# huawei-noah/xingtian

Measured on NVIDIA H100. Metric: learner env-steps/sec (Atari 84x84x4 PPO), higher is better.
Workload: dtype f32 (bf16x3 split on wgmma, fp32 accumulate in registers)

## Files before the change

include/xtb200.h:

```cpp
#ifndef XTB200_H_
#define XTB200_H_

#include <stddef.h>
#include <stdint.h>

#ifdef __cplusplus
extern "C" {
#endif

#define XTB_VERSION 101

enum xtb_status {
  XTB_OK = 0,
  XTB_ERR_ARG = -1,
  XTB_ERR_CUDA = -2,
  XTB_ERR_STATE = -3,
  XTB_ERR_NOMEM = -4
};

enum xtb_layer_kind { XTB_CONV = 0, XTB_DENSE = 1, XTB_DUELING = 2, XTB_LOGSTD = 3 };
enum xtb_act {
  XTB_ACT_NONE = 0, XTB_ACT_RELU = 1, XTB_ACT_TANH = 2, XTB_ACT_SIGMOID = 3, XTB_ACT_SOFTSIGN = 4, XTB_ACT_SOFTPLUS = 5,
  XTB_ACT_LEAKY_RELU = 6, XTB_ACT_ELU = 7, XTB_ACT_SELU = 8, XTB_ACT_SWISH = 9, XTB_ACT_GELU = 10
};
// ... 66 lines not shown
typedef struct xtb_ppo_hyper {
  float clip_ratio;
  float ent_coef;
  float vf_clip;
  float critic_coef;
} xtb_ppo_hyper;
int xtb_ppo_loss_grad(const float* logits, const float* v, const int32_t* gather_idx,
                      const int32_t* action, const float* old_logp, const float* adv,
                      const float* old_v, const float* target_v, int batch, int adim,
                      const xtb_ppo_hyper* hp, float inv_count, float* dlogits, float* dv,
                      float* loss_out, void* stream);

int xtb_vtrace_loss_grad(const float* tp_logits, const float* baseline, const float* bp_logits,
                         const int32_t* action, const uint8_t* done, const float* reward,
                         int n_traj, int step_len, int adim, float gamma, float* dlogits,
                         float* dbaseline, float* vs_out, float* pg_adv_out, float* loss_out,
                         void* stream);

int xtb_dqn_loss_grad(const float* q, const float* q_next_target, const float* q_next_online,
                      const int32_t* action, const float* reward, const uint8_t* done, int batch,
                      int adim, float gamma, float inv_count, float* dq, float* y_out,
                      float* loss_out, void* stream);

int xtb_dqn_td_loss_grad(const float* q, const float* q_next_target, const float* q_next_online, const int32_t* idx,
                         const int32_t* action, const float* reward, const uint8_t* done, const float* disc, int batch,
                         int adim, float gamma, float huber_delta, float inv_count, float* dq, float* y_out,
                         float* loss_out, void* stream);
int xtb_nstep_returns(const float* reward, const uint8_t* done, int n_env, int n_step, int n, float gamma, float* ret,
                      float* disc, int32_t* last, uint8_t* done_n, void* stream);

int xtb_mse_loss_grad(const float* q, const float* y, int batch, int adim, float inv_count, float* dq,
                      float* loss_out, void* stream);
int xtb_softmax(const float* logits, int batch, int adim, float* probs, void* stream);
int xtb_impala_keras_loss_grad(const float* logits, const float* v, const int32_t* idx, const float* action_mat,
                               const float* adv, const float* target_v, int batch, int adim, float ent_coef,
                               float value_weight, float loss_scale, float* dlogits, float* dv, float* loss_out,
                               void* stream);

typedef struct xtb_adam xtb_adam;
enum xtb_clip_mode { XTB_CLIP_NONE = 0, XTB_CLIP_GLOBAL_NORM = 1, XTB_CLIP_PER_TENSOR = 2 };
int xtb_adam_create(long long count, float lr, float beta1, float beta2, float eps, int clip_mode,
                    float clip, const long long* seg_offsets, int n_seg, float* m, float* v,
                    xtb_adam** out);
void xtb_adam_destroy(xtb_adam* opt);
int xtb_adam_step(xtb_adam* opt, float* params, const float* grads, float grad_scale, void* stream);
int xtb_adam_step_net(xtb_adam* opt, xtb_net* net, float grad_scale, void* stream);
const float* xtb_adam_grad_norm(const xtb_adam* opt);
int xtb_adam_set_lr(xtb_adam* opt, float lr);
int xtb_adam_set_decay(xtb_adam* opt, float decay);
int xtb_opt_use_rmsprop(xtb_adam* opt, float* mean_grad, float decay, float epsilon);
int xtb_opt_use_rmsprop_plain(xtb_adam* opt, float decay, float epsilon);

int xtb_ppo_heads_plan(const xtb_net* net, int pi_tensor, int v_tensor, int infer, int* kpl, int* amax);
typedef struct xtb_ppo_rollout {
  const void* obs;
  const void* action;
  const float* old_logp;
  const float* adv;
  const float* old_v;
  const float* target_v;
} xtb_ppo_rollout;
int xtb_ppo_train(xtb_net* net, xtb_adam* opt, const xtb_ppo_rollout* ro, int n_sample, int batch_size, int n_epoch,
                  const int32_t* perm, const xtb_ppo_hyper* hp, int pi_tensor, int v_tensor, int logstd_tensor,
                  float* loss_per_step, int use_graph, void* stream);

int xtb_impala_train(xtb_net* net, xtb_adam* opt, const void* obs, const int32_t* gather_idx, const float* bp_logits,
                     const int32_t* action, const uint8_t* done, const float* reward, int n_sample, int step_len,
                     float gamma, int logit_tensor, int base_tensor, float* loss_out, int use_graph, void* stream);
int xtb_dqn_train(xtb_net* net, xtb_net* target, xtb_adam* opt, const void* obs, const void* next_obs,
                  const int32_t* idx, const int32_t* action, const float* reward, const uint8_t* done,
                  const float* disc, int n_sample, float gamma, float huber_delta, int q_tensor, float* qn_t,
                  float* qn_o, float* loss_out, int use_graph, void* stream);

int xtb_impala_keras_fit(xtb_net* net, xtb_adam* opt, const void* obs, const int32_t* order, const float* action_mat,
                         const float* adv, const float* target_v, int n, int fit_batch, int logit_tensor, int v_tensor,
                         float ent_coef, float* loss_out, int use_graph, void* stream);
typedef struct xtb_impala_traj {
  const void* obs;
  const float* behav_prob;
  const float* action_mat;
  const float* reward;
  const uint8_t* done;
} xtb_impala_traj;
int xtb_impala_keras_train(xtb_net* net, xtb_adam* opt, const xtb_impala_traj* tr, int n_traj, int ep_len, int slice,
                           int fit_batch, const int32_t* order, int32_t* obs_idx, float gamma, float ent_coef,
                           int logit_tensor, int v_tensor, float* pg_adv, float* target_v, float* loss_per_slice,
                           int use_graph, void* stream);

int xtb_ppo_rollout_infer(xtb_net* net, const void* obs, const int32_t* step_idx, int n_env, int n_step, int pi_tensor,
                          int v_tensor, int logstd_tensor, uint64_t seed, unsigned long long* offset_dev, void* action,
                          float* logp, float* value, int use_graph, void* stream);

int xtb_ppo_predict_host(xtb_net* net, const void* obs_host, size_t obs_bytes, void* obs_dev, int n_env, int pi_tensor,
                         int v_tensor, int logstd_tensor, uint64_t seed, unsigned long long* offset_dev, float* out_dev,
                         float* out_host, float* head_host, int use_graph, void* stream);

int xtb_diag_gaussian_sample(const float* mean, const float* log_std, int batch, int adim, const float* normals,
                             uint64_t seed, uint64_t offset, float* action, float* logp, void* stream);
int xtb_ppo_gauss_loss_grad(const float* mean, const float* v, const float* log_std, const int32_t* gather_idx,
                            const float* action, const float* old_logp, const float* adv, const float* old_v,
                            const float* target_v, int batch, int adim, const xtb_ppo_hyper* hp, float inv_count,
                            float* dmean, float* dv, float* dlog_std, float* loss_out, void* stream);

typedef struct xtb_muzero xtb_muzero;
typedef struct xtb_muzero_desc {
  int32_t unroll;
// ... 117 lines not shown
```

xingtian_b200/capi.py:

```python
import ctypes as C
import os

HERE = os.path.dirname(os.path.abspath(__file__))
LIB_PATH = os.environ.get("XTB_LIB_PATH") or os.path.join(HERE, "lib", "libxtb200.so")

XTB_MAX_LAYERS = 16
CONV, DENSE, DUELING, LOGSTD = 0, 1, 2, 3
ACT = {None: 0, "linear": 0, "relu": 1, "tanh": 2, "sigmoid": 3, "softsign": 4, "softplus": 5, "leaky_relu": 6, "elu": 7,
       "selu": 8, "swish": 9, "gelu": 10}
CLIP_NONE, CLIP_GLOBAL_NORM, CLIP_PER_TENSOR = 0, 1, 2


class LayerDesc(C.Structure):
    _fields_ = [("kind", C.c_int32), ("src", C.c_int32), ("act", C.c_int32), ("k", C.c_int32),
                ("stride", C.c_int32), ("cout", C.c_int32), ("pad_same", C.c_int32)]


class NetDesc(C.Structure):
    _fields_ = [("input_u8", C.c_int32), ("scale", C.c_float), ("in_h", C.c_int32), ("in_w", C.c_int32),
                ("in_c", C.c_int32), ("n_layers", C.c_int32), ("layers", LayerDesc * XTB_MAX_LAYERS)]


class LayerPlan(C.Structure):
    _fields_ = [("kind", C.c_int32), ("tc", C.c_int32), ("s2d", C.c_int32), ("w_res", C.c_int32), ("n_fwd", C.c_int32),
# ... 59 lines not shown
    "xtb_net_param_count": (C.c_longlong, [_P]),
    "xtb_net_layer_params": (C.c_int, [_P, C.c_int, C.POINTER(C.c_longlong), C.POINTER(C.c_longlong),
                                       C.POINTER(C.c_int), C.POINTER(C.c_int)]),
    "xtb_net_layer_plan": (C.c_int, [_P, C.c_int, C.POINTER(LayerPlan)]),
    "xtb_net_tensor_size": (C.c_int, [_P, C.c_int]),
    "xtb_net_workspace_bytes": (C.c_size_t, [_P]),
    "xtb_net_bind": (C.c_int, [_P, _P, _P, _P, C.c_size_t]),
    "xtb_net_bind_stream": (C.c_int, [_P, _P, _P, _P, C.c_size_t, _P]),
    "xtb_net_sync_weights": (C.c_int, [_P, _P]),
    "xtb_net_tensor": (_P, [_P, C.c_int]),
    "xtb_net_tensor_grad": (_P, [_P, C.c_int]),
    "xtb_net_forward": (C.c_int, [_P, _P, _P, _P, C.c_int, _P]),
    "xtb_net_backward": (C.c_int, [_P, _P, _P, C.c_int, C.POINTER(C.c_int32), C.c_int, _P]),
    "xtb_categorical_sample": (C.c_int, [_P, C.c_int, C.c_int, _P, C.c_uint64, C.c_uint64, _P, _P, _P]),
    "xtb_argmax": (C.c_int, [_P, C.c_int, C.c_int, _P, _P]),
    "xtb_gae": (C.c_int, [_P, _P, _P, C.c_int, C.c_int, C.c_float, C.c_float, C.c_int, _P, _P, _P, _P]),
    "xtb_ppo_loss_grad": (C.c_int, [_P, _P, _P, _P, _P, _P, _P, _P, C.c_int, C.c_int, C.POINTER(PpoHyper),
                                    C.c_float, _P, _P, _P, _P]),
    "xtb_vtrace_loss_grad": (C.c_int, [_P, _P, _P, _P, _P, _P, C.c_int, C.c_int, C.c_int, C.c_float,
                                       _P, _P, _P, _P, _P, _P]),
    "xtb_dqn_loss_grad": (C.c_int, [_P, _P, _P, _P, _P, _P, C.c_int, C.c_int, C.c_float, C.c_float,
                                    _P, _P, _P, _P]),
    "xtb_dqn_td_loss_grad": (C.c_int, [_P, _P, _P, _P, _P, _P, _P, _P, C.c_int, C.c_int, C.c_float, C.c_float, C.c_float,
                                      _P, _P, _P, _P]),
    "xtb_nstep_returns": (C.c_int, [_P, _P, C.c_int, C.c_int, C.c_int, C.c_float, _P, _P, _P, _P, _P]),
    "xtb_impala_train": (C.c_int, [_P, _P, _P, _P, _P, _P, _P, _P, C.c_int, C.c_int, C.c_float, C.c_int, C.c_int, _P, C.c_int, _P]),
    "xtb_dqn_train": (C.c_int, [_P, _P, _P, _P, _P, _P, _P, _P, _P, _P, C.c_int, C.c_float, C.c_float, C.c_int, _P, _P, _P,
                               C.c_int, _P]),
    "xtb_mse_loss_grad": (C.c_int, [_P, _P, C.c_int, C.c_int, C.c_float, _P, _P, _P]),
    "xtb_softmax": (C.c_int, [_P, C.c_int, C.c_int, _P, _P]),
    "xtb_impala_keras_loss_grad": (C.c_int, [_P, _P, _P, _P, _P, _P, C.c_int, C.c_int, C.c_float, C.c_float, C.c_float,
                                             _P, _P, _P, _P]),
    "xtb_impala_keras_fit": (C.c_int, [_P, _P, _P, _P, _P, _P, _P, C.c_int, C.c_int, C.c_int, C.c_int, C.c_float, _P,
                                       C.c_int, _P]),
    "xtb_impala_keras_train": (C.c_int, [_P, _P, C.POINTER(ImpalaTraj), C.c_int, C.c_int, C.c_int, C.c_int, _P, _P,
                                         C.c_float, C.c_float, C.c_int, C.c_int, _P, _P, _P, C.c_int, _P]),
    "xtb_adam_create": (C.c_int, [C.c_longlong, C.c_float, C.c_float, C.c_float, C.c_float, C.c_int,
                                  C.c_float, C.POINTER(C.c_longlong), C.c_int, _P, _P, C.POINTER(_P)]),
    "xtb_adam_destroy": (None, [_P]),
    "xtb_adam_step": (C.c_int, [_P, _P, _P, C.c_float, _P]),
    "xtb_adam_step_net": (C.c_int, [_P, _P, C.c_float, _P]),
    "xtb_adam_grad_norm": (_P, [_P]),
    "xtb_adam_set_lr": (C.c_int, [_P, C.c_float]),
    "xtb_adam_set_decay": (C.c_int, [_P, C.c_float]),
    "xtb_opt_use_rmsprop": (C.c_int, [_P, _P, C.c_float, C.c_float]),
    "xtb_opt_use_rmsprop_plain": (C.c_int, [_P, C.c_float, C.c_float]),
    "xtb_ppo_train": (C.c_int, [_P, _P, C.POINTER(PpoRollout), C.c_int, C.c_int, C.c_int, _P, C.POINTER(PpoHyper),
                                C.c_int, C.c_int, C.c_int, _P, C.c_int, _P]),
    "xtb_ppo_rollout_infer": (C.c_int, [_P, _P, _P, C.c_int, C.c_int, C.c_int, C.c_int, C.c_int, C.c_uint64, _P, _P, _P, _P,
                                        C.c_int, _P]),
    "xtb_ppo_predict_host": (C.c_int, [_P, _P, C.c_size_t, _P, C.c_int, C.c_int, C.c_int, C.c_int, C.c_uint64, _P, _P, _P, _P,
                                       C.c_int, _P]),
    "xtb_ppo_heads_plan": (C.c_int, [_P, C.c_int, C.c_int, C.c_int, C.POINTER(C.c_int), C.POINTER(C.c_int)]),
    "xtb_diag_gaussian_sample": (C.c_int, [_P, _P, C.c_int, C.c_int, _P, C.c_uint64, C.c_uint64, _P, _P, _P]),
    "xtb_ppo_gauss_loss_grad": (C.c_int, [_P, _P, _P, _P, _P, _P, _P, _P, _P, C.c_int, C.c_int, C.POINTER(PpoHyper), C.c_float,
                                          _P, _P, _P, _P, _P]),
    "xtb_muzero_create": (C.c_int, [_P, _P, _P, C.POINTER(MuzeroDesc), C.c_int, C.POINTER(_P)]),
    "xtb_muzero_destroy": (None, [_P]),
    "xtb_muzero_train": (C.c_int, [_P, _P, C.POINTER(MuzeroBatch), C.c_int, C.c_float, _P, _P, C.c_int, _P]),
    "xtb_muzero_initial_inference": (C.c_int, [_P, _P, C.c_int, _P, _P, _P, C.c_int, _P]),
    "xtb_muzero_recurrent_inference": (C.c_int, [_P, _P, _P, C.c_int, _P, _P, _P, _P, C.c_int, _P]),
    "xtb_muzero_tree_create": (C.c_int, [_P, C.c_int, C.c_int, C.POINTER(_P)]),
    "xtb_muzero_tree_destroy": (None, [_P]),
    "xtb_muzero_search": (C.c_int, [_P, _P, _P, C.c_int, C.c_int, _P, C.c_double, C.c_double, C.c_double, C.c_double, _P, _P,
                                    C.c_int, _P]),
    "xtb_qmix_create": (C.c_int, [_P, _P, _P, C.POINTER(QmixDesc), C.POINTER(_P)]),
    "xtb_qmix_destroy": (None, [_P]),
    "xtb_qmix_train": (C.c_int, [_P, _P, _P, C.POINTER(QmixBatch), _P, C.c_int, _P]),
    "xtb_qmix_infer": (C.c_int, [_P, _P, _P, _P, _P, C.c_int, _P]),
    "xtb_scc_create": (C.c_int, [_P, _P, C.POINTER(_P), C.POINTER(SccDesc), C.POINTER(_P)]),
    "xtb_scc_destroy": (None, [_P]),
    "xtb_scc_train": (C.c_int, [_P, _P, _P, _P, C.POINTER(SccBatch), _P, C.c_int, _P]),
    "xtb_scc_infer": (C.c_int, [_P, _P, _P, _P, _P, C.c_int, _P]),
    "xtb_scc_critic": (C.c_int, [_P, _P, C.c_int, _P, C.c_int, _P]),
    "xtb_net_backward_input": (C.c_int, [_P, _P, _P, C.c_int, C.POINTER(C.c_int32), C.c_int, _P, _P]),
    "xtb_comm_unique_id": (C.c_int, [C.c_char_p, _P]),
    "xtb_comm_create": (C.c_int, [C.c_char_p, _P, C.c_int, C.c_int, C.POINTER(_P)]),
    "xtb_comm_destroy": (None, [_P]),
    "xtb_comm_world": (C.c_int, [_P]),
    "xtb_set_grad_comm": (C.c_int, [_P]),
    "xtb_comm_allreduce": (C.c_int, [_P, _P, C.c_longlong, _P]),
    "xtb_net_bench_layer": (C.c_int, [_P, C.c_int, C.c_int, _P, _P, C.c_int, _P]),
    "xtb_set_fuse_heads": (C.c_int, [C.c_int]),
    "xtb_set_tc_mode": (C.c_int, [C.c_int]),
    "xtb_get_tc_mode": (C.c_int, []),
    "xtb_tc_gemm_test": (C.c_int, [C.c_int, _P, _P, _P, C.c_int, C.c_int, C.c_int, C.c_int, _P]),
    "xtb_pinned_alloc": (_P, [C.c_size_t]),
    "xtb_pinned_free": (None, [_P]),
    "xtb_copy_h2d": (C.c_int, [_P, _P, C.c_size_t, _P]),
    "xtb_copy_h2d_staged": (C.c_int, [_P, _P, C.c_size_t, _P]),
    "xtb_copy_d2h": (C.c_int, [_P, _P, C.c_size_t, _P]),
    "xtb_stream_sync": (C.c_int, [_P]),
}

EXPORTED = tuple(_SIGS)
_lib = None


def lib():
    global _lib
    if _lib is None:
        if not os.path.exists(LIB_PATH):
            raise RuntimeError(
                "xingtian_b200: CUDA library %s is missing -- run `python -m xingtian_b200.build` "
                "(there is no CPU fallback)" % LIB_PATH)
        handle = C.CDLL(LIB_PATH)
# ... 12 lines not shown
```

xingtian_b200/csrc/bp_gemm.cuh:

```cuda
#pragma once
#include <cuda_bf16.h>
#include <cuda_runtime.h>
#include <stdint.h>

#include "gemm_f32.cuh"

#ifndef XTB_BP_WAIT_HINT
#define XTB_BP_WAIT_HINT 20000u
#endif

namespace xtb {
namespace bp {

typedef __nv_bfloat16 bf16;

__device__ __forceinline__ uint32_t smem_u32(const void* p) { return (uint32_t)__cvta_generic_to_shared(p); }
__device__ __forceinline__ void mbar_init(uint32_t bar, uint32_t count) {
  asm volatile("mbarrier.init.shared::cta.b64 [%0], %1;" ::"r"(bar), "r"(count) : "memory");
}
__device__ __forceinline__ void fence_barrier_init() { asm volatile("fence.mbarrier_init.release.cluster;" ::: "memory"); }
__device__ __forceinline__ void mbar_arrive(uint32_t bar) {
  asm volatile("mbarrier.arrive.shared::cta.b64 _, [%0];" ::"r"(bar) : "memory");
}
__device__ __forceinline__ void mbar_expect_tx(uint32_t bar, uint32_t bytes) {
// ... 737 lines not shown
            x32 += 256 >> 4; g32 += 256 >> 4;
          }
        }
        wgmma_commit();
        wgmma_wait<1>();
        if (held >= 0 && lane == 0) mbar_arrive(empty0 + 8 * held);
        held = stage;
        if (++stage == WG_STAGES) { stage = 0; phase ^= 1; }
      }
      wgmma_wait<0>();
      fence_regs<N / 2>(acc);
      if (held >= 0 && lane == 0) mbar_arrive(empty0 + 8 * held);
#pragma unroll
      for (int h = 0; h < 2; h++) {
        const int m = wg * 64 + (warp & 3) * 16 + (lane >> 2) + 8 * h;
        float* dst;
        bool ok;
        if (conv) {
          dst = a.part + (((long long)slice * a.R + r_conv) * 128 + m) * N;
          ok = true;
        } else {
          const int k = rt * 128 + m;
          dst = a.dw + (long long)k * a.ldw + nt * N;
          ok = k < a.k_rows;
        }
        if (ok) {
#pragma unroll
          for (int i = 0; i < N / 8; i++)
            *reinterpret_cast<float2*>(dst + 8 * i + 2 * q) = make_float2(acc[4 * i + 2 * h], acc[4 * i + 2 * h + 1]);
        }
      }
    }
  }
}

struct RedSeg {
  const float* part; int n_slabs; long long slab;
  int count;
  int kind;
  int N, C, KW, mts, s2d_k4;
  long long dst_off; float alpha;
  float* dst_ptr;
};
__host__ __device__ inline int s2d_real_row(int m, int k4) {
  int tap = m >> 6, ty = tap / k4, tx = tap - ty * k4;
  int dy = (m >> 4) & 3, dx = (m >> 2) & 3, c = m & 3;
  return (((4 * ty + dy) * 4 * k4 + 4 * tx + dx) << 2) + c;
}
constexpr int RED_MAX = 24;
struct RedSegs { RedSeg s[RED_MAX]; };
__global__ void __launch_bounds__(256) grad_reduce_kernel(const __grid_constant__ RedSegs segs, float* __restrict__ grads) {
  pdl_wait(); pdl_trigger();
  __shared__ float4 sh[8][32];
  const RedSeg& s = segs.s[blockIdx.y];
  if ((int)blockIdx.x * 128 >= s.count) return;
  const int lane = threadIdx.x & 31, w = threadIdx.x >> 5;
  const int i = ((int)blockIdx.x * 32 + lane) * 4;
  float4 acc = make_float4(0.f, 0.f, 0.f, 0.f);
  if (i < s.count) {
    const bool vec = ((s.count | (int)(s.slab & 3)) & 3) == 0 && (reinterpret_cast<unsigned long long>(s.part) & 15ull) == 0;
    if (vec) {
#pragma unroll 5
      for (int k = w; k < s.n_slabs; k += 8) {
        const float4 x = *reinterpret_cast<const float4*>(s.part + (long long)k * s.slab + i);
        acc.x += x.x; acc.y += x.y; acc.z += x.z; acc.w += x.w;
      }
    } else {
      for (int k = w; k < s.n_slabs; k += 8) {
        const float* p = s.part + (long long)k * s.slab + i;
        acc.x += p[0];
        if (i + 1 < s.count) acc.y += p[1];
        if (i + 2 < s.count) acc.z += p[2];
        if (i + 3 < s.count) acc.w += p[3];
      }
    }
  }
  sh[w][lane] = acc;
  __syncthreads();
  if (w != 0 || i >= s.count) return;
  float4 t = sh[0][lane];
#pragma unroll
  for (int q = 1; q < 8; q++) { const float4 x = sh[q][lane]; t.x += x.x; t.y += x.y; t.z += x.z; t.w += x.w; }
  const float v[4] = {t.x, t.y, t.z, t.w};
#pragma unroll
  for (int e = 0; e < 4; e++) {
    const int ie = i + e;
    if (ie >= s.count) break;
    long long dst;
    if (s.kind == 0) {
      const int n = ie % s.N, mm = (ie / s.N) & 127, r = ie / (s.N * 128);
      const int ky = r / s.mts, mt = r - ky * s.mts;
      const int feat = mt * 128 + mm;
      if (feat >= s.KW * s.C) continue;
      int row = ky * s.KW * s.C + feat;
      if (s.s2d_k4) row = s2d_real_row(row, s.s2d_k4);
      dst = s.dst_off + (long long)row * s.N + n;
    } else dst = s.dst_off + ie;
    (s.dst_ptr ? s.dst_ptr : grads)[dst] = s.alpha * v[e];
  }
}

__global__ void bp_split_kernel(const float* __restrict__ src, int B, int F, BpT dst) {
  pdl_wait(); pdl_trigger();
  const int b_pad = (B + 15) & ~15;
  const long long i = (long long)blockIdx.x * blockDim.x + threadIdx.x;
  const int chunks = F >> 3;
  if (i >= (long long)chunks * b_pad) return;
  const int c = (int)(i / b_pad), b = (int)(i - (long long)c * b_pad);
  uint4 hi = make_uint4(0, 0, 0, 0), lo = hi;
  if (b < B) {
// ... 196 lines not shown
```

xingtian_b200/csrc/optim.cuh:

```cuda
#pragma once
#include <cuda_bf16.h>
#include <cuda_runtime.h>
#include <stdint.h>

#include "bp_gemm.cuh"
#include "launch.cuh"

namespace xtb {

constexpr int OPT_CHUNK = 1024;
constexpr int OPT_THREADS = 256;

struct AdamState {
  float beta1_pow, beta2_pow, lr_t, grad_norm;
  unsigned int iterations;
};
struct AdamHyper {
  float lr, beta1, beta2, eps, clip;
  float decay;
};

__device__ __forceinline__ void adam_prep(AdamState* st, const AdamHyper* hyp, double* norm_sq, float* seg_scale, int n_seg,
                                          int clip_mode, float grad_scale) {
  const float clip = hyp->clip, beta1 = hyp->beta1, beta2 = hyp->beta2;
  float lr = hyp->lr;
  if (hyp->decay != 0.f) lr = lr / (1.f + hyp->decay * (float)st->iterations);
  st->iterations += 1;
  double tot = 0.0;
  for (int s = 0; s < n_seg; s++) tot += norm_sq[s];
  float gs = fabsf(grad_scale);
  float gnorm = (float)sqrt(tot) * gs;
  st->grad_norm = gnorm;
  if (clip_mode == 1) {
    float sc = clip / fmaxf(gnorm, clip);
    for (int s = 0; s < n_seg; s++) seg_scale[s] = sc * grad_scale;
  } else if (clip_mode == 2) {
    for (int s = 0; s < n_seg; s++) {
      float n = (float)sqrt(norm_sq[s]) * gs;
      seg_scale[s] = (n > clip ? clip / n : 1.f) * grad_scale;
    }
  } else {
    for (int s = 0; s < n_seg; s++) seg_scale[s] = grad_scale;
  }
  for (int s = 0; s < n_seg; s++) norm_sq[s] = 0.0;
  float b1p = st->beta1_pow * beta1, b2p = st->beta2_pow * beta2;
  st->beta1_pow = b1p; st->beta2_pow = b2p;
  st->lr_t = lr * sqrtf(1.f - b2p) / (1.f - b1p);
}

constexpr int SQN_GROUP = 4;
__global__ void __launch_bounds__(OPT_THREADS)
sqnorm_kernel(const float* __restrict__ g, const int* __restrict__ blk_seg,
              const long long* __restrict__ blk_beg, const int* __restrict__ blk_len, int n_blk,
              double* __restrict__ norm_sq, unsigned int* __restrict__ ticket, AdamState* st, const AdamHyper* __restrict__ hyp,
              float* seg_scale, int n_seg, int clip_mode, float grad_scale) {
  pdl_wait(); pdl_trigger();
  __shared__ float red[OPT_THREADS / 32];
  auto flush = [&](float s, int seg) {
#pragma unroll
    for (int o = 16; o > 0; o >>= 1) s += __shfl_xor_sync(0xffffffffu, s, o);
    if ((threadIdx.x & 31) == 0) red[threadIdx.x >> 5] = s;
    __syncthreads();
    if (threadIdx.x < 32) {
      float t = threadIdx.x < OPT_THREADS / 32 ? red[threadIdx.x] : 0.f;
#pragma unroll
      for (int o = 16; o > 0; o >>= 1) t += __shfl_xor_sync(0xffffffffu, t, o);
      if (threadIdx.x == 0) atomicAdd(norm_sq + seg, (double)t);
    }
    __syncthreads();
  };
  const int e0 = blockIdx.x * SQN_GROUP, e1 = min(e0 + SQN_GROUP, n_blk);
  float s = 0.f;
  int cur = blk_seg[e0];
  for (int e = e0; e < e1; e++) {
    if (blk_seg[e] != cur) { flush(s, cur); s = 0.f; cur = blk_seg[e]; }
    const float* p = g + blk_beg[e];
    const int n = blk_len[e];
    if ((blk_beg[e] & 3) == 0) {
      const int nv = n & ~3;
      for (int i = threadIdx.x * 4; i < nv; i += OPT_THREADS * 4) {
        const float4 v = *reinterpret_cast<const float4*>(p + i);
        s = fmaf(v.x, v.x, s); s = fmaf(v.y, v.y, s); s = fmaf(v.z, v.z, s); s = fmaf(v.w, v.w, s);
      }
      for (int i = nv + threadIdx.x; i < n; i += OPT_THREADS) { float v = p[i]; s = fmaf(v, v, s); }
    } else {
      for (int i = threadIdx.x; i < n; i += OPT_THREADS) { float v = p[i]; s = fmaf(v, v, s); }
    }
  }
  flush(s, cur);
  if (threadIdx.x == 0) {
    __threadfence();
    if (atomicAdd(ticket, 1u) == gridDim.x - 1) {
      __threadfence();
      *ticket = 0;
      adam_prep(st, hyp, norm_sq, seg_scale, n_seg, clip_mode, grad_scale);
    }
  }
}

__global__ void __launch_bounds__(OPT_THREADS)
adam_kernel(float* __restrict__ p, const float* __restrict__ g, float* __restrict__ m,
            float* __restrict__ v, const int* __restrict__ blk_seg,
            const long long* __restrict__ blk_beg, const int* __restrict__ blk_len,
            const float* __restrict__ seg_scale, const AdamState* __restrict__ st, const AdamHyper* __restrict__ hyp,
            const bp::BlobSeg* __restrict__ bsegs, int n_bsegs, __nv_bfloat16* __restrict__ w_hi, long long w_lo_off) {
  pdl_wait(); pdl_trigger();
  const float beta1 = hyp->beta1, beta2 = hyp->beta2, eps = hyp->eps;
  long long beg = blk_beg[blockIdx.x];
  int n = blk_len[blockIdx.x];
  float sc = seg_scale[blk_seg[blockIdx.x]];
  float lr_t = st->lr_t;
  const bool vec = ((beg & 3) == 0);
  int nv = vec ? (n & ~3) : 0;
  for (int i = threadIdx.x * 4; i < nv; i += OPT_THREADS * 4) {
    long long j = beg + i;
    float4 g4 = *reinterpret_cast<const float4*>(g + j);
    float4 m4 = *reinterpret_cast<const float4*>(m + j);
    float4 v4 = *reinterpret_cast<const float4*>(v + j);
    float4 p4 = *reinterpret_cast<const float4*>(p + j);
    float gg[4] = {g4.x * sc, g4.y * sc, g4.z * sc, g4.w * sc};
    float mm[4] = {m4.x, m4.y, m4.z, m4.w}, vv[4] = {v4.x, v4.y, v4.z, v4.w}, pp[4] = {p4.x, p4.y, p4.z, p4.w};
#pragma unroll
    for (int q = 0; q < 4; q++) {
      mm[q] = beta1 * mm[q] + (1.f - beta1) * gg[q];
      vv[q] = beta2 * vv[q] + (1.f - beta2) * gg[q] * gg[q];
      pp[q] -= lr_t * mm[q] / (sqrtf(vv[q]) + eps);
    }
    *reinterpret_cast<float4*>(m + j) = make_float4(mm[0], mm[1], mm[2], mm[3]);
    *reinterpret_cast<float4*>(v + j) = make_float4(vv[0], vv[1], vv[2], vv[3]);
    *reinterpret_cast<float4*>(p + j) = make_float4(pp[0], pp[1], pp[2], pp[3]);
    if (w_hi) bp::blob_store4(bsegs, n_bsegs, w_hi, w_lo_off, j, pp);
  }
  for (int i = nv + threadIdx.x; i < n; i += OPT_THREADS) {
    long long j = beg + i;
    float gg = g[j] * sc;
    float mm = beta1 * m[j] + (1.f - beta1) * gg;
    float vv = beta2 * v[j] + (1.f - beta2) * gg * gg;
    m[j] = mm; v[j] = vv;
    float pn = p[j] - lr_t * mm / (sqrtf(vv) + eps);
// ... 60 lines not shown
```

xingtian_b200/csrc/xtb_engine.cu:

```cuda
#include "../../include/xtb200.h"

#include <cuda_runtime.h>

#include <atomic>
#include <cmath>
#include <cstdarg>
#include <cstdio>
#include <cstring>
#include <map>
#include <memory>
#include <string>
#include <tuple>
#include <vector>

#include "gemm_f32.cuh"
#include "optim.cuh"
#include "rl_kernels.cuh"
#include "qmix.cuh"
#include "scc.cuh"
#include "stager.cuh"
#include "bp_gemm.cuh"
#include "comm.cuh"
#include <cstdlib>
#include <type_traits>

using namespace xtb;

static thread_local std::string g_err;
static std::atomic<long long> g_launches{0};

static int fail(int code, const char* fmt, ...) {
  char buf[512];
  va_list ap;
  va_start(ap, fmt);
  vsnprintf(buf, sizeof buf, fmt, ap);
  va_end(ap);
  g_err = buf;
  return code;
}
#define CUDA_TRY(x)                                                                          \
  do {                                                                                       \
    cudaError_t e_ = (x);                                                                    \
    if (e_ != cudaSuccess)                                                                   \
      return fail(XTB_ERR_CUDA, "%s:%d %s -> %s", __FILE__, __LINE__, #x, cudaGetErrorString(e_)); \
  } while (0)
#define LAUNCH_CHECK()                                                                       \
  do {                                                                                       \
    g_launches.fetch_add(1, std::memory_order_relaxed);                                      \
    cudaError_t e_ = cudaPeekAtLastError();                                                  \
    if (e_ != cudaSuccess)                                                                   \
      return fail(XTB_ERR_CUDA, "%s:%d launch -> %s", __FILE__, __LINE__, cudaGetErrorString(e_)); \
  } while (0)

extern "C" int xtb_version(void) { return XTB_VERSION; }
extern "C" const char* xtb_last_error(void) { return g_err.c_str(); }
extern "C" long long xtb_launch_count(void) { return g_launches.load(); }
// ... 1118 lines not shown
    if (rc) return rc;
    XLAUNCH(dueling_dgrad_kernel, (B + 7) / 8, 256, 0, st, (const float*)gout_f32(net, t), (const float*)out_f32(net, s),
            (const float*)out_f32(net, s2), B, lp.out_size, lp.src_act, lp.adv_act, acc, acc2, gout_f32(net, s), gout_f32(net, s2));
    LAUNCH_CHECK();
    wrote(net, s, true, kF32); wrote(net, s2, true, kF32);
    return XTB_OK;
  }
  if (use_tc(lp)) {
    int rc = ensure_bp(net, t, B, true, st);
    if (rc) return rc;
    if (dgrad_act(lp) != 0) { rc = ensure_bp(net, s, B, false, st); if (rc) return rc; }
    if (acc) { rc = ensure_bp(net, s, B, true, st); if (rc) return rc; }
    float* dbp = fuse_db ? (float*)(net->ws + lp.dbpart_off) : nullptr;
    cudaError_t te = tc_dgrad(net, i, B, acc, dbp, st);
    if (te != cudaSuccess) return fail(XTB_ERR_CUDA, "tensor-core dgrad launch (layer %d): %s", i, cudaGetErrorString(te));
    LAUNCH_CHECK();
    if (fuse_db) {
      const int units = lp.d.kind == XTB_CONV ? lp.q.H * lp.q.W : lp.K / lp.n_dg;
      queue_reduction(net, dbp, std::min(kSMs, units * ((B + 127) / 128)), lp.n_dg, lp.n_dg, net->L[s - 1].b_off);
    }
    wrote(net, s, true, kPlanes);
    return XTB_OK;
  }
  int rc = ensure_f32(net, t, B, true, st);
  if (rc) return rc;
  rc = ensure_f32(net, s, B, false, st);
  if (rc) return rc;
  if (acc) { rc = ensure_f32(net, s, B, true, st); if (rc) return rc; }
  const float* dy = gout_f32(net, t);
  const float* x = out_f32(net, s);
  float* gsrc = gout_f32(net, s);
  const float* w = net->params + lp.w_off;
  if (lp.d.kind == XTB_CONV) {
    const ConvTabs tab = conv_tabs(net, lp);
    ADgrad al{dy, lp.g, tab.dkyx, tab.dco, lp.sshift};
    BConvDgrad bl{w, tab.wk, lp.N};
    EpiDgrad ep{gsrc, x, dgrad_act(lp), lp.g.C, acc, nullptr, 0};
    launch_gemm(al, bl, ep, B * lp.g.H * lp.g.W, lp.g.C, lp.Kd, false, st);
  } else {
    ADense<float> al{dy, nullptr, lp.N};
    BTransposed bl{w, lp.N};
    EpiDgrad ep{gsrc, x, dgrad_act(lp), lp.K, acc, nullptr, 0};
    launch_gemm(al, bl, ep, B, lp.K, lp.N, false, st);
  }
  LAUNCH_CHECK();
  wrote(net, s, true, kF32);
  return XTB_OK;
}

static int flush_reductions(xtb_net* net, cudaStream_t st) {
  if (net->pending.empty()) return XTB_OK;
  bp::RedSegs segs;
  memset(&segs, 0, sizeof segs);
  int mx = 0;
  if (net->pending.size() > bp::RED_MAX) return fail(XTB_ERR_STATE, "too many pending reductions");
  for (size_t k = 0; k < net->pending.size(); k++) { segs.s[k] = net->pending[k]; mx = std::max(mx, net->pending[k].count); }
  dim3 grid((mx + 127) / 128, (unsigned)net->pending.size());
  XLAUNCH(bp::grad_reduce_kernel, grid, 256, 0, st, segs, net->grads);
  LAUNCH_CHECK();
  net->pending.clear();
  return XTB_OK;
}

static int net_forward_impl(xtb_net* net, const float* params, const void* obs, const int32_t* gather_idx,
                            int batch, void* stream, unsigned skip_mask, unsigned want_f32_mask, int split_rows = 0);
extern "C" int xtb_net_forward(xtb_net* net, const float* params, const void* obs, const int32_t* gather_idx,
                               int batch, void* stream) {
  return net_forward_impl(net, params, obs, gather_idx, batch, stream, 0u, ~0u);
}
static int net_forward_impl(xtb_net* net, const float* params, const void* obs, const int32_t* gather_idx,
                            int batch, void* stream, unsigned skip_mask, unsigned want_f32_mask, int split_rows) {
  if (!net || !net->ws) return fail(XTB_ERR_STATE, "xtb_net_forward: net not bound");
  if (batch <= 0 || batch > net->max_batch) return fail(XTB_ERR_ARG, "batch %d out of range (max %d)", batch, net->max_batch);
  if (!obs) return fail(XTB_ERR_ARG, "obs is null");
  const float* P = params ? params : net->params;
  const bool tc_allowed = (P == net->params);
  cudaStream_t st = S(stream);
  const int nl = (int)net->L.size();
  invalidate(net, true, false);
  for (int i = 0; i < nl; i++) {
    if (skip_mask & (1u << i)) continue;
    const LayerPlan& lp = net->L[i];
    bool direct = lp.d.kind == XTB_DENSE && ((want_f32_mask >> (i + 1)) & 1u);
    if (lp.d.kind == XTB_DENSE)
      for (int j = i + 1; j < nl; j++)
        if (reads(net->L[j], i + 1) && !(skip_mask & (1u << j)) && !(tc_allowed && use_tc(net->L[j]))) direct = true;
    int rc = op_forward(net, i, P, tc_allowed, obs, gather_idx, batch, split_rows ? split_rows : batch, direct, st);
    if (rc) return rc;
  }
  for (int t = 1; t <= nl; t++) {
    if (!((want_f32_mask >> t) & 1u) || (skip_mask & (1u << (t - 1))) || net->tsize[t] == 0) continue;
    int rc = ensure_f32(net, t, batch, false, st);
    if (rc) return rc;
  }
  return XTB_OK;
}

struct BackwardOpts {
  const int32_t* heads; int n_heads;
  unsigned heads_bp = 0u;
  unsigned heads_dy = 0u;
  unsigned skip = 0u;
  bool zero_grads = true;
  unsigned bias_done = 0u;
  float* dobs = nullptr;
  bool all_reduce = false;
  BackwardOpts(const int32_t* h, int n) : heads(h), n_heads(n) {}
};
static int net_backward_impl(xtb_net* net, const void* obs, const int32_t* gather_idx, int batch, void* stream,
                             const BackwardOpts& o);
extern "C" int xtb_net_backward(xtb_net* net, const void* obs, const int32_t* gather_idx, int batch,
                                const int32_t* head_tensors, int n_heads, void* stream) {
  return net_backward_impl(net, obs, gather_idx, batch, stream, BackwardOpts(head_tensors, n_heads));
}
static int input_grad_check(const xtb_net* net) {
  if (net->desc.input_u8 || net->desc.scale != 1.f) return fail(XTB_ERR_ARG, "input gradient: the observation must be float with scale 1");
  for (const auto& lp : net->L)
    if (lp.d.src == 0 && lp.d.kind != XTB_DENSE && lp.d.kind != XTB_LOGSTD)
      return fail(XTB_ERR_ARG, "input gradient: only dense layers may read the observation");
  return XTB_OK;
}
extern "C" int xtb_net_backward_input(xtb_net* net, const void* obs, const int32_t* gather_idx, int batch,
                                      const int32_t* head_tensors, int n_heads, float* dobs, void* stream) {
  if (!obs || !dobs || !head_tensors) return fail(XTB_ERR_ARG, "xtb_net_backward_input: null pointer");
  BackwardOpts o(head_tensors, n_heads); o.dobs = dobs;
  return net_backward_impl(net, obs, gather_idx, batch, stream, o);
}
static int net_backward_impl(xtb_net* net, const void* obs, const int32_t* gather_idx, int batch, void* stream,
                             const BackwardOpts& o) {
  if (!net || !net->ws || !net->grads) return fail(XTB_ERR_STATE, "xtb_net_backward: net not bound (grads required)");
  if (batch <= 0 || batch > net->max_batch) return fail(XTB_ERR_ARG, "batch out of range");
  if (o.dobs) { int rc = input_grad_check(net); if (rc) return rc; }
  cudaStream_t st = S(stream);
  xtb_comm* comm = o.all_reduce ? g_comm : nullptr;
  const int nl = (int)net->L.size();
  std::vector<char> has_grad(nl + 1, 0), written(nl + 1, 0);
  std::vector<char> dy(nl + 1, 0);
  long long early_off = 0, early_cnt = 0;
  invalidate(net, false, true);
  if (o.zero_grads) net->pending.clear();
  for (int h = 0; h < o.n_heads; h++) {
    int t = o.heads[h];
    if (t < 1 || t > nl || net->tsize[t] == 0) return fail(XTB_ERR_ARG, "bad head tensor %d", t);
    has_grad[t] = 1; written[t] = 1; dy[t] = (o.heads_dy >> t) & 1u;
    wrote(net, t, true, (o.heads_bp >> t) & 1u ? kPlanes : kF32);
  }
  if (o.zero_grads) CUDA_TRY(cudaMemsetAsync(net->grads, 0, net->n_params * sizeof(float), st));
  std::vector<char> fuse_bias(nl + 1, 0);
  for (int s = 1; s <= nl; s++) {
    if (o.bias_done & (1u << s)) { fuse_bias[s] = 2; continue; }
    const LayerPlan& ps = net->L[s - 1];
    if (act_is_ext(ps.d.act)) continue;
    int consumers = 0, cj = -1;
    for (int j = 0; j < nl; j++) if (reads(net->L[j], s) && !(o.skip & (1u << j))) { consumers++; cj = j; }
    if (consumers != 1) continue;
    const LayerPlan& c = net->L[cj];
    if (!use_tc(c)) continue;
    if (ps.d.kind == XTB_CONV ? c.n_dg == ps.N : (c.d.kind == XTB_DENSE && c.n_dg == ps.N && c.K == ps.N)) fuse_bias[s] = 1;
  }
  for (int i = nl - 1; i >= 0; i--) {
    if (o.skip & (1u << i)) continue;
    const LayerPlan& lp = net->L[i];
    int t = i + 1;
    if (!has_grad[t]) continue;
    const bool act_bwd = dy[t] && act_is_ext(lp.d.act);
    if (act_bwd) { int rc = act_backward(net, t, batch, st); if (rc) return rc; }
    int rc = op_wgrad(net, i, obs, gather_idx, batch, st, fuse_bias[t] != 0 || act_bwd);
    if (rc) return rc;
    if (comm && comm->world > 1 && early_cnt == 0 && lp.d.kind == XTB_DENSE && use_tc(lp) && (long long)lp.K * lp.N >= (1 << 16)) {
      early_off = lp.w_off; early_cnt = (long long)lp.K * lp.N;
      rc = comm_fork_allreduce(comm, net->grads + early_off, early_cnt, st);
      if (rc) return rc;
    }
    if (lp.d.kind == XTB_DUELING) {
      const int s = lp.d.src, s2 = lp.d.k;
      rc = op_dgrad(net, i, written[s] ? 1 : 0, batch, st, false, written[s2] ? 1 : 0);
      if (rc) return rc;
      written[s] = written[s2] = 1; has_grad[s] = has_grad[s2] = 1;
    } else if (lp.d.src != 0) {
      int s = lp.d.src;
      rc = op_dgrad(net, i, written[s] ? 1 : 0, batch, st, fuse_bias[s] == 1);
      if (rc) return rc;
      written[s] = 1; has_grad[s] = 1; dy[s] = 1;
    }
  }
  if (o.dobs) {
    bool first = true;
    for (int i = 0; i < nl; i++) {
      const LayerPlan& lp = net->L[i];
      if (lp.d.src != 0 || lp.d.kind != XTB_DENSE || (o.skip & (1u << i))) continue;
      if (!has_grad[i + 1]) continue;
      int rc = ensure_f32(net, i + 1, batch, true, st);
      if (rc) return rc;
      ADense<float> al{(const float*)gout_f32(net, i + 1), nullptr, lp.N};
      BTransposed bl{net->params + lp.w_off, lp.N};
      EpiDgrad ep{o.dobs, o.dobs, 0, lp.K, first ? 0 : 1, nullptr, 0};
      launch_gemm(al, bl, ep, batch, lp.K, lp.N, false, st);
      LAUNCH_CHECK();
      first = false;
    }
    if (first) CUDA_TRY(cudaMemsetAsync(o.dobs, 0, (size_t)batch * net->tsize[0] * sizeof(float), st));
  }
  int rc = flush_reductions(net, st);
  if (rc || !comm || comm->world == 1) return rc;
  if (early_cnt == 0) return xtb_comm_allreduce(comm, net->grads, net->n_params, stream);
  int nrc = g_nccl.GroupStart();
  if (!nrc && early_off > 0) nrc = g_nccl.AllReduce(net->grads, net->grads, (size_t)early_off, kNcclFloat, kNcclSum, comm->comm, st);
  const long long tail = net->n_params - (early_off + early_cnt);
  if (!nrc && tail > 0)
    nrc = g_nccl.AllReduce(net->grads + early_off + early_cnt, net->grads + early_off + early_cnt, (size_t)tail, kNcclFloat, kNcclSum, comm->comm, st);
  int erc = g_nccl.GroupEnd();
// ... 406 lines not shown
    cudaGraphDestroy(graph);
    if (e != cudaSuccess) return fail(XTB_ERR_CUDA, "graph instantiate failed: %s", cudaGetErrorString(e));
    if (g_graphs.size() >= kMaxCachedGraphs) {
      for (auto& kv : g_graphs) cudaGraphExecDestroy(kv.second.exec);
      g_graphs.clear();
    }
    it = g_graphs.emplace(key, GraphVal{exec, captured}).first;
  }
  CUDA_TRY(cudaGraphLaunch(it->second.exec, sc.st));
  g_launches.fetch_add(it->second.kernels, std::memory_order_relaxed);
  g_graph_replays.fetch_add(1, std::memory_order_relaxed);
  return sc.end();
}

template <class STEP>
static int ppo_epoch_loop(xtb_net* net, xtb_adam* opt, int N, int B, int E, const int32_t* perm, float* loss_per_step,
                          void* stream, STEP&& minibatch) {
  int steps_per_epoch = (N + B - 1) / B;
  CUDA_TRY(cudaMemsetAsync(loss_per_step, 0, sizeof(float) * E * steps_per_epoch, S(stream)));
  int step = 0;
  for (int e = 0; e < E; e++) {
    for (int s0 = 0; s0 < N; s0 += B, step++) {
      int mb = std::min(B, N - s0);
      int rc = minibatch(perm + (long long)e * N + s0, mb, loss_per_step + step);
      if (rc) return rc;
      rc = xtb_adam_step_net(opt, net, 1.f, stream);
      if (rc) return rc;
    }
  }
  return XTB_OK;
}

static float dp_inv_world() { return g_comm ? 1.f / g_comm->world : 1.f; }

static int learner_check(const char* fn, bool missing, const xtb_net* net, const xtb_adam* opt, long long rows, bool dp_ok,
                         long long max_rows = 0, long long n_params = 0) {
  if (missing) return fail(XTB_ERR_ARG, "%s: null pointer", fn);
  if (!net->ws || !net->grads) return fail(XTB_ERR_STATE, "%s: net not bound", fn);
  if (!dp_ok && g_comm) return fail(XTB_ERR_STATE, "%s: data-parallel training (communicator) is not supported", fn);
  if (opt && opt->count != (n_params ? n_params : net->n_params))
    return fail(XTB_ERR_ARG, "%s: optimiser/net size mismatch (%lld != %lld)", fn, opt->count, n_params ? n_params : net->n_params);
  if (!max_rows) max_rows = net->max_batch;
  if (rows < 1 || rows > max_rows) return fail(XTB_ERR_ARG, "%s: batch %lld not in [1, %lld]", fn, rows, max_rows);
  return XTB_OK;
}

static bool ppo_heads_fusable(const xtb_net* net, int pi_t, int v_t, bool infer) {
  const LayerPlan& lpi = net->L[pi_t - 1];
  const LayerPlan& lv = net->L[v_t - 1];
  return g_fuse_heads && lpi.d.kind == XTB_DENSE && lv.d.kind == XTB_DENSE && lpi.d.act == 0 && lv.d.act == 0 &&
         lpi.d.src != 0 && lv.d.src != 0 && lpi.K == lv.K && heads_fit(lpi.K, net->tsize[pi_t], infer);
}

template <class LOSS>
static int heads_fused(xtb_net* net, const void* obs, PpoHeadsArgs& a, int mb, int pi_t, int v_t, unsigned skip,
                       long long ls_off, float* loss_dst, void* stream) {
  const LayerPlan& lpi = net->L[pi_t - 1];
  const LayerPlan& lv = net->L[v_t - 1];
  const int adim = net->tsize[pi_t];
  const int32_t* idx = a.idx;
  CUDA_TRY(cudaMemsetAsync(net->grads, 0, net->n_params * sizeof(float), S(stream)));
  net->pending.clear();
  a.h_pi = out_f32(net, lpi.d.src); a.h_v = out_f32(net, lv.d.src);
  a.g_pi = gout_f32(net, lpi.d.src); a.g_v = gout_f32(net, lv.d.src);
  const bool ext_pi = act_is_ext(lpi.src_act), ext_v = act_is_ext(lv.src_act);
  const bool bp_pi = use_tc(net->L[lpi.d.src - 1]) && net->plane_elems[lpi.d.src] > 0 && !ext_pi;
  const bool bp_v = use_tc(net->L[lv.d.src - 1]) && net->plane_elems[lv.d.src] > 0 && !ext_v;
  a.gp_hi = bp_pi ? gout_bp(net, lpi.d.src).hi : nullptr; a.gp_lo = net->plane_elems[lpi.d.src];
  a.gv_hi = bp_v ? gout_bp(net, lv.d.src).hi : nullptr; a.gv_lo = net->plane_elems[lv.d.src];
  a.pitch = net->pitch;
  a.w_pi = net->params + lpi.w_off; a.b_pi = net->params + lpi.b_off; a.w_v = net->params + lv.w_off; a.b_v = net->params + lv.b_off;
  auto only_feeds_heads = [&](int tsr) { for (int j = 0; j < (int)net->L.size(); j++) if (reads(net->L[j], tsr) && !(skip & (1u << j))) return false; return true; };
  bool bh_pi_ok = net->L[lpi.d.src - 1].d.kind == XTB_DENSE && only_feeds_heads(lpi.d.src) && !ext_pi;
  bool bh_v_ok = net->L[lv.d.src - 1].d.kind == XTB_DENSE && only_feeds_heads(lv.d.src) && !ext_v;
  a.B = mb; a.K = lpi.K; a.A = adim; a.act_pi = dgrad_act(lpi); a.act_v = dgrad_act(lv); a.shared = lpi.d.src == lv.d.src ? 1 : 0;
  int blocks = std::max(1, std::min(kSMs, (mb + 7) / 8));
  const int HK = lpi.K, nacc = HK * adim + 3 * HK + adim + 2 + (LOSS::kLogStd ? adim : 0);
  a.part = (float*)(net->ws + net->heads_part_off); a.slab = (nacc + 3) & ~3;
  size_t shb = (size_t)8 * nacc * sizeof(float);
  { cudaError_t ea = ensure_kernel_attrs(); if (ea != cudaSuccess) return fail(XTB_ERR_CUDA, "kernel attributes: %s", cudaGetErrorString(ea)); }
  XLAUNCH(heads_pick(kHeadsKernels<LOSS>, a.K, a.A)->kern, blocks, 256, shb, S(stream), a);
  LAUNCH_CHECK();
  {
    auto seg = [&](int off, int count, long long dst_off, float* dst_ptr = nullptr) {
      queue_reduction(net, a.part + off, blocks, a.slab, count, dst_off, dst_ptr);
    };
    seg(0, HK * adim, lpi.w_off);
    seg(HK * adim, HK, lv.w_off);
    if (bh_pi_ok) seg(HK * adim + HK, HK, net->L[lpi.d.src - 1].b_off);
    if (!a.shared && bh_v_ok) seg(HK * adim + 2 * HK, HK, net->L[lv.d.src - 1].b_off);
    seg(HK * adim + 3 * HK, adim, lpi.b_off);
    seg(HK * adim + 3 * HK + adim, 1, lv.b_off);
    seg(HK * adim + 3 * HK + adim + 1, 1, 0, loss_dst);
    if (LOSS::kLogStd) seg(HK * adim + 3 * HK + adim + 2, adim, ls_off);
  }
  const int32_t srcs[2] = {lpi.d.src, lv.d.src};
  BackwardOpts o(srcs, a.shared ? 1 : 2);
  o.heads_bp = (bp_pi ? (1u << lpi.d.src) : 0u) | (bp_v ? (1u << lv.d.src) : 0u);
  o.heads_dy = (ext_pi ? (1u << lpi.d.src) : 0u) | (ext_v ? (1u << lv.d.src) : 0u);
  o.bias_done = (bh_pi_ok ? (1u << lpi.d.src) : 0u) | ((lpi.d.src != lv.d.src && bh_v_ok) ? (1u << lv.d.src) : 0u);
  o.skip = skip; o.zero_grads = false; o.all_reduce = true;
  return net_backward_impl(net, obs, idx, mb, stream, o);
}

template <class DIST>
static int ppo_train_launch(xtb_net* net, xtb_adam* opt, const xtb_ppo_rollout* ro, int N, int B, int E, const int32_t* perm,
                            const xtb_ppo_hyper* hp, int pi_t, int v_t, int ls_t, float* loss_per_step, float inv_world,
                            void* stream) {
  const int32_t heads[2] = {pi_t, v_t};
  const auto* action = static_cast<const typename DIST::Action*>(ro->action);
  const int adim = net->tsize[pi_t];
  const long long ls_off = DIST::kLogStd ? net->L[ls_t - 1].w_off : -1;
  const LayerPlan& lpi = net->L[pi_t - 1];
  const LayerPlan& lv = net->L[v_t - 1];
  const bool fuse = ppo_heads_fusable(net, pi_t, v_t, false);
  const unsigned skip = fuse ? ((1u << (pi_t - 1)) | (1u << (v_t - 1))) : 0u;
  return ppo_epoch_loop(net, opt, N, B, E, perm, loss_per_step, stream, [&](const int32_t* idx, int mb, float* step_loss) -> int {
    const unsigned want = fuse ? ((1u << lpi.d.src) | (1u << lv.d.src)) : ((1u << pi_t) | (1u << v_t));
    int rc = net_forward_impl(net, nullptr, ro->obs, idx, mb, stream, skip, want);
    if (rc) return rc;
    if (fuse) {
      PpoHeadsArgs a;
      memset(&a, 0, sizeof a);
      a.idx = idx; a.old_logp = ro->old_logp; a.adv = ro->adv; a.old_v = ro->old_v; a.target_v = ro->target_v;
      if constexpr (DIST::kLogStd) { a.action_f = action; a.log_std = net->params + ls_off; }
      else a.action = action;
      a.logits_out = xtb_net_tensor(net, pi_t); a.v_out = xtb_net_tensor(net, v_t);
// ... 1112 lines not shown
```

Baseline: 288,100.

## Skip grad memset when fused PPO step overwrites every gradient, flatten reductions

Adds a static analysis that checks whether the fused PPO heads step plus backward pass assigns every gradient element exactly once, and if so drops the full cudaMemsetAsync of the gradient buffer. The grad reduction kernel moves from a 2D grid padded to the largest segment to a 1D grid that walks segment block counts, so no empty blocks are launched. The squared-norm kernel gets an unrolled fast path for full aligned chunk groups. The memset skip depends on the coverage analysis being right; if any element is missed, stale gradients leak into the update.

```diff
diff --git a/include/xtb200.h b/include/xtb200.h
--- a/include/xtb200.h
+++ b/include/xtb200.h
@@ -142,6 +142,7 @@
 int xtb_opt_use_rmsprop_plain(xtb_adam* opt, float decay, float epsilon);
 
 int xtb_ppo_heads_plan(const xtb_net* net, int pi_tensor, int v_tensor, int infer, int* kpl, int* amax);
+int xtb_ppo_grads_assigned(const xtb_net* net, int pi_tensor, int v_tensor, int* assigned);
 typedef struct xtb_ppo_rollout {
   const void* obs;
   const void* action;
diff --git a/xingtian_b200/capi.py b/xingtian_b200/capi.py
--- a/xingtian_b200/capi.py
+++ b/xingtian_b200/capi.py
@@ -135,6 +135,7 @@
     "xtb_ppo_predict_host": (C.c_int, [_P, _P, C.c_size_t, _P, C.c_int, C.c_int, C.c_int, C.c_int, C.c_uint64, _P, _P, _P, _P,
                                        C.c_int, _P]),
     "xtb_ppo_heads_plan": (C.c_int, [_P, C.c_int, C.c_int, C.c_int, C.POINTER(C.c_int), C.POINTER(C.c_int)]),
+    "xtb_ppo_grads_assigned": (C.c_int, [_P, C.c_int, C.c_int, C.POINTER(C.c_int)]),
     "xtb_diag_gaussian_sample": (C.c_int, [_P, _P, C.c_int, C.c_int, _P, C.c_uint64, C.c_uint64, _P, _P, _P]),
     "xtb_ppo_gauss_loss_grad": (C.c_int, [_P, _P, _P, _P, _P, _P, _P, _P, _P, C.c_int, C.c_int, C.POINTER(PpoHyper), C.c_float,
                                           _P, _P, _P, _P, _P]),
diff --git a/xingtian_b200/csrc/bp_gemm.cuh b/xingtian_b200/csrc/bp_gemm.cuh
--- a/xingtian_b200/csrc/bp_gemm.cuh
+++ b/xingtian_b200/csrc/bp_gemm.cuh
@@ -813,10 +813,11 @@
 __global__ void __launch_bounds__(256) grad_reduce_kernel(const __grid_constant__ RedSegs segs, float* __restrict__ grads) {
   pdl_wait(); pdl_trigger();
   __shared__ float4 sh[8][32];
-  const RedSeg& s = segs.s[blockIdx.y];
-  if ((int)blockIdx.x * 128 >= s.count) return;
+  int y = 0, bx = (int)blockIdx.x;
+  for (int c; bx >= (c = (segs.s[y].count + 127) / 128); y++) bx -= c;
+  const RedSeg& s = segs.s[y];
   const int lane = threadIdx.x & 31, w = threadIdx.x >> 5;
-  const int i = ((int)blockIdx.x * 32 + lane) * 4;
+  const int i = (bx * 32 + lane) * 4;
   float4 acc = make_float4(0.f, 0.f, 0.f, 0.f);
   if (i < s.count) {
     const bool vec = ((s.count | (int)(s.slab & 3)) & 3) == 0 && (reinterpret_cast<unsigned long long>(s.part) & 15ull) == 0;
diff --git a/xingtian_b200/csrc/optim.cuh b/xingtian_b200/csrc/optim.cuh
--- a/xingtian_b200/csrc/optim.cuh
+++ b/xingtian_b200/csrc/optim.cuh
@@ -72,19 +72,33 @@
   const int e0 = blockIdx.x * SQN_GROUP, e1 = min(e0 + SQN_GROUP, n_blk);
   float s = 0.f;
   int cur = blk_seg[e0];
-  for (int e = e0; e < e1; e++) {
-    if (blk_seg[e] != cur) { flush(s, cur); s = 0.f; cur = blk_seg[e]; }
-    const float* p = g + blk_beg[e];
-    const int n = blk_len[e];
-    if ((blk_beg[e] & 3) == 0) {
-      const int nv = n & ~3;
-      for (int i = threadIdx.x * 4; i < nv; i += OPT_THREADS * 4) {
-        const float4 v = *reinterpret_cast<const float4*>(p + i);
-        s = fmaf(v.x, v.x, s); s = fmaf(v.y, v.y, s); s = fmaf(v.z, v.z, s); s = fmaf(v.w, v.w, s);
+  static_assert(OPT_CHUNK == 4 * OPT_THREADS, "a full chunk is one float4 per thread");
+  bool fast = e1 - e0 == SQN_GROUP && blk_seg[e1 - 1] == cur && (blk_beg[e0] & 3) == 0;
+#pragma unroll
+  for (int q = 0; q < SQN_GROUP; q++) fast = fast && blk_len[e0 + q] == OPT_CHUNK;
+  if (fast) {
+    float4 v[SQN_GROUP];
+#pragma unroll
+    for (int q = 0; q < SQN_GROUP; q++) v[q] = *reinterpret_cast<const float4*>(g + blk_beg[e0] + q * OPT_CHUNK + threadIdx.x * 4);
+#pragma unroll
+    for (int q = 0; q < SQN_GROUP; q++) {
+      s = fmaf(v[q].x, v[q].x, s); s = fmaf(v[q].y, v[q].y, s); s = fmaf(v[q].z, v[q].z, s); s = fmaf(v[q].w, v[q].w, s);
+    }
+  } else {
+    for (int e = e0; e < e1; e++) {
+      if (blk_seg[e] != cur) { flush(s, cur); s = 0.f; cur = blk_seg[e]; }
+      const float* p = g + blk_beg[e];
+      const int n = blk_len[e];
+      if ((blk_beg[e] & 3) == 0) {
+        const int nv = n & ~3;
+        for (int i = threadIdx.x * 4; i < nv; i += OPT_THREADS * 4) {
+          const float4 v = *reinterpret_cast<const float4*>(p + i);
+          s = fmaf(v.x, v.x, s); s = fmaf(v.y, v.y, s); s = fmaf(v.z, v.z, s); s = fmaf(v.w, v.w, s);
+        }
+        for (int i = nv + threadIdx.x; i < n; i += OPT_THREADS) { float v = p[i]; s = fmaf(v, v, s); }
+      } else {
+        for (int i = threadIdx.x; i < n; i += OPT_THREADS) { float v = p[i]; s = fmaf(v, v, s); }
       }
-      for (int i = nv + threadIdx.x; i < n; i += OPT_THREADS) { float v = p[i]; s = fmaf(v, v, s); }
-    } else {
-      for (int i = threadIdx.x; i < n; i += OPT_THREADS) { float v = p[i]; s = fmaf(v, v, s); }
     }
   }
   flush(s, cur);
diff --git a/xingtian_b200/csrc/xtb_engine.cu b/xingtian_b200/csrc/xtb_engine.cu
--- a/xingtian_b200/csrc/xtb_engine.cu
+++ b/xingtian_b200/csrc/xtb_engine.cu
@@ -2,6 +2,7 @@
 
 #include <cuda_runtime.h>
 
+#include <algorithm>
 #include <atomic>
 #include <cmath>
 #include <cstdarg>
@@ -1226,11 +1227,11 @@
   if (net->pending.empty()) return XTB_OK;
   bp::RedSegs segs;
   memset(&segs, 0, sizeof segs);
-  int mx = 0;
+  int blocks = 0;
   if (net->pending.size() > bp::RED_MAX) return fail(XTB_ERR_STATE, "too many pending reductions");
-  for (size_t k = 0; k < net->pending.size(); k++) { segs.s[k] = net->pending[k]; mx = std::max(mx, net->pending[k].count); }
-  dim3 grid((mx + 127) / 128, (unsigned)net->pending.size());
-  XLAUNCH(bp::grad_reduce_kernel, grid, 256, 0, st, segs, net->grads);
+  for (size_t k = 0; k < net->pending.size(); k++) { segs.s[k] = net->pending[k]; blocks += (net->pending[k].count + 127) / 128; }
+  if (blocks == 0) { net->pending.clear(); return XTB_OK; }
+  XLAUNCH(bp::grad_reduce_kernel, blocks, 256, 0, st, segs, net->grads);
   LAUNCH_CHECK();
   net->pending.clear();
   return XTB_OK;
@@ -1281,6 +1282,16 @@
   bool all_reduce = false;
   BackwardOpts(const int32_t* h, int n) : heads(h), n_heads(n) {}
 };
+static bool bias_fused_into_consumer(const xtb_net* net, int s, unsigned skip) {
+  const LayerPlan& ps = net->L[s - 1];
+  if (act_is_ext(ps.d.act)) return false;
+  int consumers = 0, cj = -1;
+  for (int j = 0; j < (int)net->L.size(); j++) if (reads(net->L[j], s) && !(skip & (1u << j))) { consumers++; cj = j; }
+  if (consumers != 1) return false;
+  const LayerPlan& c = net->L[cj];
+  if (!use_tc(c)) return false;
+  return ps.d.kind == XTB_CONV ? c.n_dg == ps.N : (c.d.kind == XTB_DENSE && c.n_dg == ps.N && c.K == ps.N);
+}
 static int net_backward_impl(xtb_net* net, const void* obs, const int32_t* gather_idx, int batch, void* stream,
                              const BackwardOpts& o);
 extern "C" int xtb_net_backward(xtb_net* net, const void* obs, const int32_t* gather_idx, int batch,
@@ -1322,15 +1333,8 @@
   if (o.zero_grads) CUDA_TRY(cudaMemsetAsync(net->grads, 0, net->n_params * sizeof(float), st));
   std::vector<char> fuse_bias(nl + 1, 0);
   for (int s = 1; s <= nl; s++) {
-    if (o.bias_done & (1u << s)) { fuse_bias[s] = 2; continue; }
-    const LayerPlan& ps = net->L[s - 1];
-    if (act_is_ext(ps.d.act)) continue;
-    int consumers = 0, cj = -1;
-    for (int j = 0; j < nl; j++) if (reads(net->L[j], s) && !(o.skip & (1u << j))) { consumers++; cj = j; }
-    if (consumers != 1) continue;
-    const LayerPlan& c = net->L[cj];
-    if (!use_tc(c)) continue;
-    if (ps.d.kind == XTB_CONV ? c.n_dg == ps.N : (c.d.kind == XTB_DENSE && c.n_dg == ps.N && c.K == ps.N)) fuse_bias[s] = 1;
+    if (o.bias_done & (1u << s)) fuse_bias[s] = 2;
+    else if (bias_fused_into_consumer(net, s, o.skip)) fuse_bias[s] = 1;
   }
   for (int i = nl - 1; i >= 0; i--) {
     if (o.skip & (1u << i)) continue;
@@ -1843,6 +1847,70 @@
          lpi.d.src != 0 && lv.d.src != 0 && lpi.K == lv.K && heads_fit(lpi.K, net->tsize[pi_t], infer);
 }
 
+static bool heads_take_bias(const xtb_net* net, int tsr, unsigned skip) {
+  if (net->L[tsr - 1].d.kind != XTB_DENSE) return false;
+  for (int j = 0; j < (int)net->L.size(); j++) if (reads(net->L[j], tsr) && !(skip & (1u << j))) return false;
+  return true;
+}
+
+static bool conv_reduction_is_onto(const LayerPlan& lp) {
+  std::vector<char> hit(lp.K, 0);
+  const int feats = lp.q.KW * lp.q.C;
+  for (int r = 0; r < lp.R; r++)
+    for (int mm = 0; mm < 128; mm++) {
+      const int ky = r / lp.mts, feat = (r - ky * lp.mts) * 128 + mm;
+      if (feat >= feats) continue;
+      int row = ky * feats + feat;
+      if (lp.s2d) row = bp::s2d_real_row(row, lp.k4);
+      if (row < 0 || row >= lp.K || hit[row]) return false;
+      hit[row] = 1;
+    }
+  return std::count(hit.begin(), hit.end(), 1) == lp.K;
+}
+
+static bool fused_step_assigns_grads(const xtb_net* net, int pi_t, int v_t) {
+  if (!ppo_heads_fusable(net, pi_t, v_t, false)) return false;
+  const int nl = (int)net->L.size();
+  const LayerPlan& lpi = net->L[pi_t - 1];
+  const LayerPlan& lv = net->L[v_t - 1];
+  const unsigned skip = (1u << (pi_t - 1)) | (1u << (v_t - 1));
+  std::vector<std::pair<long long, long long>> w;
+  auto put = [&](long long off, long long n) { w.emplace_back(off, off + n); };
+  put(lpi.w_off, (long long)lpi.K * lpi.N); put(lpi.b_off, lpi.N);
+  put(lv.w_off, (long long)lv.K * lv.N); put(lv.b_off, lv.N);
+  std::vector<char> has_grad(nl + 1, 0);
+  has_grad[lpi.d.src] = has_grad[lv.d.src] = 1;
+  for (int i = nl - 1; i >= 0; i--) {
+    if (skip & (1u << i)) continue;
+    const LayerPlan& lp = net->L[i];
+    const int t = i + 1;
+    if (lp.d.kind != XTB_CONV && lp.d.kind != XTB_DENSE) return false;
+    if (!has_grad[t] || !use_tc(lp) || act_is_ext(lp.d.act)) return false;
+    if (lp.d.kind == XTB_CONV && !conv_reduction_is_onto(lp)) return false;
+    put(lp.w_off, (long long)lp.K * lp.N);
+    const bool by_heads = (t == lpi.d.src || t == lv.d.src) && heads_take_bias(net, t, skip);
+    if (!by_heads && !bias_fused_into_consumer(net, t, skip)) return false;
+    put(lp.b_off, lp.N);
+    if (lp.d.src != 0) has_grad[lp.d.src] = 1;
+  }
+  std::sort(w.begin(), w.end());
+  long long end = 0;
+  for (const auto& r : w) {
+    if (r.first != end) return false;
+    end = r.second;
+  }
+  return end == net->n_params;
+}
+
+static int ppo_heads_check(const char* fn, const xtb_net* net, int pi_t, int v_t, int ls_t);
+extern "C" int xtb_ppo_grads_assigned(const xtb_net* net, int pi_t, int v_t, int* assigned) {
+  const char* fn = "xtb_ppo_grads_assigned";
+  if (!net || !assigned) return fail(XTB_ERR_ARG, "%s: null pointer", fn);
+  if (int rc = ppo_heads_check(fn, net, pi_t, v_t, 0)) return rc;
+  *assigned = fused_step_assigns_grads(net, pi_t, v_t) ? 1 : 0;
+  return XTB_OK;
+}
+
 template <class LOSS>
 static int heads_fused(xtb_net* net, const void* obs, PpoHeadsArgs& a, int mb, int pi_t, int v_t, unsigned skip,
                        long long ls_off, float* loss_dst, void* stream) {
@@ -1850,7 +1918,8 @@
   const LayerPlan& lv = net->L[v_t - 1];
   const int adim = net->tsize[pi_t];
   const int32_t* idx = a.idx;
-  CUDA_TRY(cudaMemsetAsync(net->grads, 0, net->n_params * sizeof(float), S(stream)));
+  if (!fused_step_assigns_grads(net, pi_t, v_t))
+    CUDA_TRY(cudaMemsetAsync(net->grads, 0, net->n_params * sizeof(float), S(stream)));
   net->pending.clear();
   a.h_pi = out_f32(net, lpi.d.src); a.h_v = out_f32(net, lv.d.src);
   a.g_pi = gout_f32(net, lpi.d.src); a.g_v = gout_f32(net, lv.d.src);
@@ -1861,9 +1930,8 @@
   a.gv_hi = bp_v ? gout_bp(net, lv.d.src).hi : nullptr; a.gv_lo = net->plane_elems[lv.d.src];
   a.pitch = net->pitch;
   a.w_pi = net->params + lpi.w_off; a.b_pi = net->params + lpi.b_off; a.w_v = net->params + lv.w_off; a.b_v = net->params + lv.b_off;
-  auto only_feeds_heads = [&](int tsr) { for (int j = 0; j < (int)net->L.size(); j++) if (reads(net->L[j], tsr) && !(skip & (1u << j))) return false; return true; };
-  bool bh_pi_ok = net->L[lpi.d.src - 1].d.kind == XTB_DENSE && only_feeds_heads(lpi.d.src) && !ext_pi;
-  bool bh_v_ok = net->L[lv.d.src - 1].d.kind == XTB_DENSE && only_feeds_heads(lv.d.src) && !ext_v;
+  const bool bh_pi_ok = heads_take_bias(net, lpi.d.src, skip) && !ext_pi;
+  const bool bh_v_ok = heads_take_bias(net, lv.d.src, skip) && !ext_v;
   a.B = mb; a.K = lpi.K; a.A = adim; a.act_pi = dgrad_act(lpi); a.act_v = dgrad_act(lv); a.shared = lpi.d.src == lv.d.src ? 1 : 0;
   int blocks = std::max(1, std::min(kSMs, (mb + 7) / 8));
   const int HK = lpi.K, nacc = HK * adim + 3 * HK + adim + 2 + (LOSS::kLogStd ? adim : 0);
```

Result: no change. 290,400, median of 6 (+0.8%).
